# Juzhan/TAP-Net

Hardware: AMD Instinct MI355X
Metric: env-steps/s (batch placements) 2D n=10 LB_GREEDY; 1/2/4/8 GPU + CPU ref (higher is better)
Workload: dtype i32 height-maps / f64 candidate scores / f32 masks

## Files before the change

### tap-net_amd/csrc/tap_masks.h

```cpp
#pragma once

#include <hip/hip_runtime.h>

#include <cstdint>
#include <type_traits>
#include <cstdlib>

#include "tap_stream_variant.h"

constexpr size_t TAP_WT_MAX_BYTES = 64u << 20;

struct MaskArgs {
    int B, n, R, nR, rows, update_rows, static_rows;
    const float *dyn_in;
    float *dyn_out;
    const float *static_;
    const int64_t *ptr;
    const float *mask_in;
    const float *cs_in;
    float *cs_out;
    float *cur_out;
    float *mask_out;
    const unsigned long long *bits_in;
    unsigned long long *bits_out;
    int *nonbinary;
    int c4_magic, rp;
    int wt;
    int sb_mul, sb_add, nq, nq2;
    int inplace;
};

inline int tap_write_through(size_t bytes);

constexpr int TAP_HOT_MAGIC_MASK = 0xffffff, TAP_HOT_SB_MUL_SHIFT = 24, TAP_HOT_SB_ADD_SHIFT = 26, TAP_HOT_SB_MASK = 3;

inline MaskArgs mask_finish(MaskArgs a)
{
    const int c4 = a.nR >> 2;
    a.c4_magic = c4 > 0 ? 65536 / c4 + 1 : 0;
    static_assert(65536 + 1 <= TAP_HOT_MAGIC_MASK, "c4_magic shares its kernel argument with sb_mul / sb_add (TAP_MASK_HOT_ARGS)");
    a.rp = c4 > 0 ? 64 / c4 : 0;
    a.wt = tap_write_through((size_t)a.B * a.rows * a.nR * sizeof(float));
    const bool al = a.wt && c4 > 0 && ((a.rp * c4) & 3) == 0;
    a.sb_mul = al ? (a.rows * c4) & 3 : 0;
    a.sb_add = al ? (int)((reinterpret_cast<uintptr_t>(a.dyn_out) >> 4) & 3) : 0;
    a.nq = a.rp > 0 ? (a.rows + a.rp - 1) / a.rp : 0;
    a.nq2 = a.rp > 0 ? (2 * a.rows + a.rp - 1) / a.rp : 0;
    return a;
}

struct LaneRole {
    int rsub, c4;
    int r0;
    int nq;
    int sb;
};

__device__ __forceinline__ LaneRole stream_lane_role(int lane, int env, int C4, int RP, int c4_magic, int sb_mul, int sb_add, int nq)
{
    const int sb = __builtin_amdgcn_readfirstlane((env * sb_mul + sb_add) & 3);
    int role = lane - sb;
    const bool late = role < 0;
    role += late ? RP * C4 : 0;
    LaneRole o;
    o.rsub = (int)(((unsigned)role * (unsigned)c4_magic) >> 16);
    o.c4 = role - o.rsub * C4;
    o.r0 = o.rsub - (late ? RP : 0);
    o.nq = nq + (sb != 0);
    o.sb = sb;
    return o;
}

__host__ __device__ __forceinline__ bool mask_builds_bits(const MaskArgs &a) { return !a.bits_in && a.bits_out && a.dyn_in; }

#define TAP_MASK_HOT_PARAMS const int64_t *h_ptr, const float *h_static, const float *h_mask_in, const void *h_src, int h_B, \
                            int h_nR, int h_static_rows, int h_c4_magic
#define TAP_MASK_HOT_NAMES h_ptr, h_static, h_mask_in, h_src, h_B, h_nR, h_static_rows, h_c4_magic
#define TAP_MASK_HOT_ARGS(m) (m).ptr, (m).static_, (m).mask_in,                                                              \
        ((m).bits_in ? static_cast<const void *>((m).bits_in) : static_cast<const void *>((m).dyn_in)), (m).B, (m).nR,       \
        (m).static_rows, ((m).c4_magic | (((m).sb_mul & TAP_HOT_SB_MASK) << TAP_HOT_SB_MUL_SHIFT) |                           \
                          (((m).sb_add & TAP_HOT_SB_MASK) << TAP_HOT_SB_ADD_SHIFT))
__device__ __forceinline__ MaskArgs tap_mask_hot(const MaskArgs &k, bool src_is_bits, TAP_MASK_HOT_PARAMS)
{
    MaskArgs m = k;
    m.ptr = h_ptr; m.static_ = h_static; m.mask_in = h_mask_in;
    m.B = h_B; m.nR = h_nR; m.static_rows = h_static_rows; m.c4_magic = h_c4_magic & TAP_HOT_MAGIC_MASK;
    m.sb_mul = (h_c4_magic >> TAP_HOT_SB_MUL_SHIFT) & TAP_HOT_SB_MASK; m.sb_add = (h_c4_magic >> TAP_HOT_SB_ADD_SHIFT) & TAP_HOT_SB_MASK;
    if (src_is_bits) m.bits_in = static_cast<const unsigned long long *>(h_src);
    else m.dyn_in = static_cast<const float *>(h_src);
    return m;
}


#ifdef TAP_PROF
constexpr int TAP_PROF_WGS = 2048, TAP_PROF_WAVES = 16;
static __device__ unsigned long long tap_prof_tl[TAP_PROF_WGS * TAP_PROF_WAVES * 4];
#define TL_STAMP(i) do { if ((threadIdx.x & 63) == 0 && blockIdx.x < TAP_PROF_WGS) \
        tap_prof_tl[(blockIdx.x * TAP_PROF_WAVES + (threadIdx.x >> 6)) * 4 + (i)] = __builtin_amdgcn_s_memrealtime(); } while (0)
#define TL_WAIT_VM() __builtin_amdgcn_s_waitcnt(0)
#else
#define TL_STAMP(i) do { } while (0)
#define TL_WAIT_VM() do { } while (0)
#endif

__device__ __forceinline__ void tap_wave_lds_sync_m()
{
    __builtin_amdgcn_fence(__ATOMIC_RELEASE, "wavefront");
    __builtin_amdgcn_wave_barrier();
    __builtin_amdgcn_fence(__ATOMIC_ACQUIRE, "wavefront");
}

__device__ __forceinline__ void store_stream(float4 *dst, const float4 &v, int wt)
{
    typedef float v4f __attribute__((ext_vector_type(4)));
    const v4f nv = {v.x, v.y, v.z, v.w};
    if (wt) asm volatile("global_store_dwordx4 %0, %1, off sc0 sc1\n\ts_nop 1" : : "v"(dst), "v"(nv) : "memory");
    else __builtin_nontemporal_store(nv, reinterpret_cast<v4f *>(dst));
}

inline int tap_write_through(size_t bytes, size_t limit)
{
    static const int forced = [] { const char *e = getenv("TAP_WRITE_THROUGH"); return e ? (e[0] != '0') : -1; }();
    if (forced >= 0) return forced;
    return bytes <= limit;
}
inline int tap_write_through(size_t bytes) { return tap_write_through(bytes, TAP_WT_MAX_BYTES); }

__device__ __forceinline__ float bit_as_float(unsigned long long w, int r)
{
    const unsigned half = r < 32 ? (unsigned)w : (unsigned)(w >> 32);
    return (float)((half >> (r & 31)) & 1u);
}

__device__ __forceinline__ long tap_mod_col(long p, int n, int nR)
{
    if ((unsigned long)p >= (unsigned long)nR) p = 0;
    while (p >= n) p -= n;
    return p;
}

__device__ __forceinline__ void mask_column(const MaskArgs &a, int env, int j, long real_m,
                                            float move, float small, float large)
{
    float keep = a.mask_in ? a.mask_in[(size_t)env * a.nR + j] : 1.f;
    if (a.ptr)
        for (int r = 0; r < a.R; ++r)
            if (j == real_m + (long)a.n * r) keep = 0.f;
    if (a.mask_out) a.mask_out[(size_t)env * a.nR + j] = keep;
    const float dm = small * large + move;
    if (a.cur_out) a.cur_out[(size_t)env * a.nR + j] = dm != 0.f ? 0.f : keep;
}


struct ClearRanges {
    int lo[3], hi[3];
};

__device__ __forceinline__ ClearRanges clear_ranges(const MaskArgs &a, long real)
{
    ClearRanges c;
    for (int i = 0; i < 3; ++i) {
        const long r = real + (long)a.n * i;
        const bool on = i < a.update_rows && real >= 0 && r < a.rows;
        c.lo[i] = on ? (int)(r * a.nR) : -1;
        c.hi[i] = on ? (int)((r + 1) * a.nR) : -1;
    }
    return c;
}

__device__ __forceinline__ bool in_cleared(const ClearRanges &c, int f)
{
    return (f >= c.lo[0] && f < c.hi[0]) || (f >= c.lo[1] && f < c.hi[1]) || (f >= c.lo[2] && f < c.hi[2]);
}

__device__ __forceinline__ void mask_env(const MaskArgs &a, int env, int lane, long real, long p)
{
    const int nR = a.nR;
    const size_t slab = (size_t)a.rows * nR;
    const long real_m = (p >= 0 && p < nR) ? tap_mod_col(p, a.n, a.nR) : -1 - (long)a.n * a.R;
    for (int j = lane; j < nR; j += 64) {
        float sum[3], row[3];
#pragma unroll
        for (int s = 0; s < 3; ++s) {
            sum[s] = a.cs_in[((size_t)env * 3 + s) * nR + j];
            const long r = real + (long)a.n * s;
            row[s] = (a.dyn_out && s < a.update_rows && real >= 0 && r < a.rows)
                         ? a.dyn_in[(size_t)env * slab + (size_t)r * nR + j] : 0.f;
        }
#pragma unroll
        for (int s = 0; s < 3; ++s) {
            sum[s] -= row[s];
            if (a.cs_out) a.cs_out[((size_t)env * 3 + s) * nR + j] = sum[s];
        }
        mask_column(a, env, j, real_m, sum[0], sum[1], sum[2]);
    }
}

template <int NS, int U, int NC>
__device__ __forceinline__ void stream_wave_fast(const MaskArgs &a, int senv0, int lane,
                                                 const bool (&on)[NS], float *lds)
{
    const int nR = a.nR;
    const size_t slab = (size_t)a.rows * nR;
    const int nchunk = (int)(slab / 4);
    int total = 0;
#pragma unroll
    for (int k = 0; k < NS; ++k) if (on[k]) total = (k + 1) * nchunk;
    if (total == 0) return;
    long p[NS];
    float row0[NS][NC], cs[NS][NC][3], keep[NS][NC];
#pragma unroll
    for (int k = 0; k < NS; ++k) {
        const int env = senv0 + k;
        p[k] = on[k] ? (long)a.ptr[env] : 0;
#pragma unroll
        for (int c = 0; c < NC; ++c) {
            const int j = lane + 64 * c;
            const bool ok = on[k] && j < nR;
            row0[k][c] = ok ? a.static_[(size_t)env * a.static_rows * nR + j] : 0.f;
            keep[k][c] = ok ? (a.mask_in ? a.mask_in[(size_t)env * nR + j] : 1.f) : 0.f;
#pragma unroll
            for (int s = 0; s < 3; ++s) cs[k][c][s] = ok ? a.cs_in[((size_t)env * 3 + s) * nR + j] : 0.f;
        }
    }
    for (int i = lane; i < NS * 3 * nR; i += 64) lds[i] = 0.f;

    const float4 *s4 = reinterpret_cast<const float4 *>(a.dyn_in + (size_t)senv0 * slab);
    float4 *d4 = reinterpret_cast<float4 *>(a.dyn_out + (size_t)senv0 * slab);
    ClearRanges cr[NS];
    bool have_real = false;
    for (int base = 0; base < total; base += 64 * U) {
        float4 v[U];
#pragma unroll
        for (int u = 0; u < U; ++u) v[u] = s4[min(base + u * 64 + lane, total - 1)];
        if (!have_real) {
#pragma unroll
            for (int k = 0; k < NS; ++k) {
                float r0 = -1.f;
#pragma unroll
                for (int c = 0; c < NC; ++c) {
                    const float t = __shfl(row0[k][c], (int)(p[k] & 63));
                    if ((p[k] >> 6) == c && p[k] >= 0 && p[k] < nR) r0 = t;
                }
                cr[k] = clear_ranges(a, on[k] ? (long)r0 : -1);
            }
            have_real = true;
        }
#pragma unroll
        for (int u = 0; u < U; ++u) {
            const int q = base + u * 64 + lane;
            if (q < total) {
                const int k = (NS > 1 && q >= nchunk) ? 1 : 0;
                const int f = (q - k * nchunk) * 4;
#pragma unroll
                for (int s = 0; s < 3; ++s)
                    if (f >= cr[k].lo[s] && f < cr[k].hi[s]) {
                        *reinterpret_cast<float4 *>(lds + (k * 3 + s) * nR + (f - cr[k].lo[s])) = v[u];
                        v[u] = make_float4(0.f, 0.f, 0.f, 0.f);
                    }
                d4[q] = v[u];
            }
        }
    }
    __builtin_amdgcn_fence(__ATOMIC_RELEASE, "wavefront");
    __builtin_amdgcn_wave_barrier();
    __builtin_amdgcn_fence(__ATOMIC_ACQUIRE, "wavefront");
#pragma unroll
    for (int k = 0; k < NS; ++k) {
        if (!on[k]) continue;
        const int env = senv0 + k;
        const long real_m = (p[k] >= 0 && p[k] < nR) ? tap_mod_col(p[k], a.n, a.nR) : -1 - (long)a.n * a.R;
#pragma unroll
        for (int c = 0; c < NC; ++c) {
            const int j = lane + 64 * c;
            if (j >= nR) continue;
            float sum[3];
#pragma unroll
            for (int s = 0; s < 3; ++s) {
                sum[s] = cs[k][c][s] - lds[(k * 3 + s) * nR + j];
                if (a.cs_out) a.cs_out[((size_t)env * 3 + s) * nR + j] = sum[s];
            }
            float kp = keep[k][c];
            for (int r = 0; r < a.R; ++r)
                if (j == real_m + (long)a.n * r) kp = 0.f;
            if (a.mask_out) a.mask_out[(size_t)env * nR + j] = kp;
            const float dm = sum[1] * sum[2] + sum[0];
            if (a.cur_out) a.cur_out[(size_t)env * nR + j] = dm != 0.f ? 0.f : kp;
        }
    }
}

template <int NS>
__device__ __forceinline__ void stream_build_bits(const MaskArgs &a, int senv0, int lane, const bool (&on)[NS],
                                                  unsigned long long *tile )
{
    typedef unsigned long long u64;
    const int nR = a.nR, C4 = nR >> 2, rows = a.rows;
    const int rsub = (int)(((unsigned)lane * (unsigned)a.c4_magic) >> 16), c4 = lane - rsub * C4, RP = a.rp;
    for (int i = lane; i < NS * nR; i += 64) tile[i] = 0ull;
    tap_wave_lds_sync_m();
    int bad = 0;
    constexpr int U = 4;
    for (int r0 = rsub; r0 < rows; r0 += U * RP) {
        float4 v[NS][U];
#pragma unroll
        for (int k = 0; k < NS; ++k) {
            const float4 *src = reinterpret_cast<const float4 *>(a.dyn_in + (size_t)(senv0 + (on[k] ? k : 0)) * rows * nR) + c4;
#pragma unroll
            for (int u = 0; u < U; ++u) v[k][u] = src[(size_t)min(r0 + u * RP, rows - 1) * C4];
        }
#pragma unroll
        for (int k = 0; k < NS; ++k) {
            unsigned lo[4] = {0u, 0u, 0u, 0u}, hi[4] = {0u, 0u, 0u, 0u};
#pragma unroll
            for (int u = 0; u < U; ++u) {
                const int r = r0 + u * RP;
                if (r >= rows || rsub >= RP || !on[k]) continue;
                const float e[4] = {v[k][u].x, v[k][u].y, v[k][u].z, v[k][u].w};
#pragma unroll
                for (int q = 0; q < 4; ++q) {
                    const unsigned nz = e[q] != 0.f;
                    bad += (nz && e[q] != 1.f);
                    if (r < 32) lo[q] |= nz << r; else hi[q] |= nz << (r - 32);
                }
            }
            if (on[k] && rsub < RP) {
#pragma unroll
                for (int q = 0; q < 4; ++q) {
                    const u64 word = ((u64)hi[q] << 32) | lo[q];
                    if (word) atomicOr(&tile[k * nR + c4 * 4 + q], word);
                }
            }
        }
    }
    if (a.nonbinary) {
        const unsigned long long any = __ballot(bad != 0);
        if (any) {
#pragma unroll
            for (int o = 32; o > 0; o >>= 1) bad += __shfl_xor(bad, o);
            if (lane == 0) atomicAdd(a.nonbinary, bad);
        }
    }
    tap_wave_lds_sync_m();
}

__device__ __forceinline__ int tap_mod_small(int v, int n)
{
#pragma unroll
    for (int r = 0; r < 5; ++r) v = v >= n ? v - n : v;
    while (v >= n) v -= n;
    return v;
}

template <int NS, int NC, bool BUILD = false, bool MERGED = true, int C4S = 0, bool INPLACE = false, bool FULL = false>
__device__ __forceinline__ void stream_wave_bits_r4(const MaskArgs &a, int senv0, int lane, const bool (&on_)[NS],
                                                 float *lds = nullptr)
{
    static_assert(!(BUILD && INPLACE), "the first step on a fresh tensor writes all of it");
    bool on[NS];
#pragma unroll
    for (int k = 0; k < NS; ++k) on[k] = FULL ? true : on_[k];
#if defined(TAP_STREAM_LOAD_BJ)
    constexpr bool BJ_X = false;
#elif defined(TAP_STREAM_BJX_ALL)
    constexpr bool BJ_X = !BUILD && NC == 1 && (C4S == 5 || C4S == 15);
#else
    constexpr bool BJ_X = !BUILD && NC == 1 && NS == 1 && (C4S == 5 || C4S == 15);
#endif
    typedef unsigned long long u64;
    static_assert(NS <= 2, "a stream wave expands one or two slabs");
    if (!on[0]) return;
    const int nR = C4S ? 4 * C4S : a.nR, C4 = C4S ? C4S : nR >> 2, rows = C4S ? (C4S == 10 ? 60 : 30) : a.rows, n = C4S ? (C4S == 10 ? 20 : 10) : a.n;
    const int RP = C4S ? 64 / C4S : a.rp;
    const int c4_magic = C4S ? 65536 / C4S + 1 : a.c4_magic;
    const bool lane_on = lane < RP * C4;
#ifdef TAP_STREAM_UNALIGNED
    const LaneRole role = stream_lane_role(lane, 0, C4, RP, c4_magic, 0, 0, 0);
#else
    const LaneRole role = stream_lane_role(lane, senv0, C4, RP, c4_magic, a.sb_mul, a.sb_add, 0);
#endif
    const bool first_row = role.rsub == 0;
    u64 *tile = reinterpret_cast<u64 *>(lds);
    const void *any = BUILD ? static_cast<const void *>(a.dyn_in) : static_cast<const void *>(a.bits_in);
    const bool has_ptr = FULL || a.ptr != nullptr, has_static = FULL || a.static_ != nullptr, has_mask = FULL || a.mask_in != nullptr;
    const int64_t *ptrp = has_ptr ? a.ptr : static_cast<const int64_t *>(any);
    const float *stp = has_static ? a.static_ : static_cast<const float *>(any);
    const float *mip = has_mask ? a.mask_in : static_cast<const float *>(any);
    long praw[NS];
    float row0[NS][NC], keep[NS][NC];
    u64 bj[NS][NC];
    ulonglong2 w[NS][2];
#pragma unroll
    for (int k = 0; k < NS; ++k) {
        const int env = on[k] ? senv0 + k : senv0;
        praw[k] = ptrp[has_ptr ? env : 0];
        const float *strow = stp + (has_static ? (size_t)env * a.static_rows * nR : (size_t)0);
        const float *mirow = mip + (has_mask ? (size_t)env * nR : (size_t)0);
#pragma unroll
        for (int c = 0; c < NC; ++c) {
            const unsigned j = (unsigned)min(lane + 64 * c, nR - 1);
            row0[k][c] = strow[has_static ? j : 0u];
            keep[k][c] = mirow[has_mask ? j : 0u];
        }
    }
#ifdef TAP_STREAM_G2
    __builtin_amdgcn_s_waitcnt(0x0F70);
#endif
    if (!BUILD) {
#pragma unroll
        for (int k = 0; k < NS; ++k) {
            const int env = on[k] ? senv0 + k : senv0;
            const unsigned long long *brow = a.bits_in + (size_t)env * nR;
            if constexpr (!BJ_X) {
#pragma unroll
                for (int c = 0; c < NC; ++c) bj[k][c] = brow[(unsigned)min(lane + 64 * c, nR - 1)];
            }
            const ulonglong2 *src = reinterpret_cast<const ulonglong2 *>(brow) + (unsigned)(role.c4 * 2);
            w[k][0] = src[0];
            w[k][1] = src[1];
        }
    }
    if (BUILD) {
        stream_build_bits<NS>(a, senv0, lane, on, tile);
#pragma unroll
        for (int k = 0; k < NS; ++k) {
#pragma unroll
            for (int c = 0; c < NC; ++c) bj[k][c] = tile[(size_t)k * nR + min(lane + 64 * c, nR - 1)];
            const ulonglong2 *src = reinterpret_cast<const ulonglong2 *>(tile + (size_t)k * nR + role.c4 * 4);
            w[k][0] = src[0];
            w[k][1] = src[1];
        }
    }
    float *o_dyn = a.dyn_out, *o_cur = a.cur_out, *o_mask = a.mask_out;
    unsigned long long *o_bits = a.bits_out;
    int o_wt = a.wt;
#ifdef TAP_STREAM_EARLY_ARGS
    asm volatile("" : "+s"(o_dyn), "+s"(o_cur), "+s"(o_mask), "+s"(o_bits), "+s"(o_wt));
#endif
    __builtin_amdgcn_s_waitcnt(0x0F70);
#ifdef TAP_PROF
    TL_STAMP(1);
#endif
    const u64 nmask = (n >= 64) ? ~0ull : ((1ull << n) - 1ull);
    auto mod_n = [&](int v) -> int {
        if constexpr (C4S != 0) return (int)((unsigned)v % (unsigned)(C4S == 10 ? 20 : 10));
        else return tap_mod_small(v, n);
    };
    int jm[NC];
#pragma unroll
    for (int c = 0; c < NC; ++c) jm[c] = mod_n(min(lane + 64 * c, nR - 1));
    u64 clr[NS];
    int pm[NS], realk[NS];
    constexpr int UR_C = C4S != 0 ? 3 : 0;
    const int ur = UR_C ? UR_C : a.update_rows;
#pragma unroll
    for (int k = 0; k < NS; ++k) {
        const bool valid_v = on[k] && has_ptr && praw[k] >= 0 && praw[k] < nR;
#ifdef TAP_STREAM_VPICK
        constexpr bool SPICK = false;
#else
        constexpr bool SPICK = NS > 1;
#endif
        bool valid;
        int p, real;
        if constexpr (!SPICK) {
            valid = valid_v;
            p = valid ? (int)praw[k] : 0;
            float r0 = -1.f;
#pragma unroll
            for (int c = 0; c < NC; ++c) {
                const float t = __shfl(row0[k][c], p & 63);
                if (valid && has_static && (p >> 6) == c) r0 = t;
            }
            real = (r0 > -1.f && r0 < (float)rows) ? (int)r0 : -1;
        } else {
            const int ps = __builtin_amdgcn_readfirstlane(valid_v ? (int)praw[k] : -1);
            valid = ps >= 0;
            p = valid ? ps : 0;
            float r0 = -1.f;
#pragma unroll
            for (int c = 0; c < NC; ++c) {
                const float t = __int_as_float(__builtin_amdgcn_readlane(__float_as_int(row0[k][c]), p & 63));
                if (valid && has_static && (p >> 6) == c) r0 = t;
            }
            real = __builtin_amdgcn_readfirstlane((r0 > -1.f && r0 < (float)rows) ? (int)r0 : -1);
        }
        u64 m = 0;
#pragma unroll
        for (int i = 0; i < 3; ++i) {
            const int r = real + n * i;
            if (i < ur && real >= 0 && r < rows) m |= 1ull << r;
        }
        clr[k] = m;
        realk[k] = real;
        pm[k] = valid ? mod_n(p) : -1;
    }
    u64 nw[NS][4];
#pragma unroll
    for (int k = 0; k < NS; ++k) {
        nw[k][0] = w[k][0].x & ~clr[k]; nw[k][1] = w[k][0].y & ~clr[k];
        nw[k][2] = w[k][1].x & ~clr[k]; nw[k][3] = w[k][1].y & ~clr[k];
    }
    if constexpr (INPLACE) {
        if (o_dyn) {
            const float4 z = make_float4(0.f, 0.f, 0.f, 0.f);
            const int total = ur * C4;
            for (int idx = lane; idx < total; idx += 64) {
                const int i = (idx * c4_magic) >> 16, c = idx - i * C4;
#pragma unroll
                for (int k = 0; k < NS; ++k) {
                    const int r = realk[k] + n * i;
                    if (!on[k] || realk[k] < 0 || r >= rows) continue;
                    float4 *dst = reinterpret_cast<float4 *>(o_dyn) + ((size_t)(senv0 + k) * rows + r) * C4 + c;
#if defined(TAP_INPLACE_STORE) && TAP_INPLACE_STORE == 1
                    store_stream(dst, z, o_wt);
#elif defined(TAP_INPLACE_STORE) && TAP_INPLACE_STORE == 2
                    *dst = z;
#else
                    if (o_wt) store_stream(dst, z, 1); else *dst = z;
#endif
                }
            }
        }
    }
    if (lane_on) {
        if (!INPLACE && o_dyn) {
            const int non = (NS > 1 && on[NS - 1]) ? 2 : 1;
            const int total = non * rows;
            const int nq = (C4S ? (non * rows + RP - 1) / RP : (non > 1 ? a.nq2 : a.nq)) + role.nq;
            float4 *dst = reinterpret_cast<float4 *>(o_dyn + (size_t)senv0 * rows * nR) + role.c4;
            int rr = role.r0;
            bool done = false;
            if constexpr (NS > 1 && !MERGED) {
                if (rows <= 32) {
#pragma unroll
                    for (int k = 0; k < NS; ++k) {
                        if (!on[k]) continue;
                        float4 *dk = dst + (size_t)k * rows * C4;
                        const unsigned m0 = (unsigned)nw[k][0], m1 = (unsigned)nw[k][1], m2 = (unsigned)nw[k][2], m3 = (unsigned)nw[k][3];
                        for (int r = role.rsub; r < rows; r += RP) {
                            const float4 v = make_float4((float)((m0 >> r) & 1u), (float)((m1 >> r) & 1u),
                                                         (float)((m2 >> r) & 1u), (float)((m3 >> r) & 1u));
                            store_stream(&dk[(size_t)r * C4], v, o_wt);
                        }
                    }
                    done = true;
                }
            }
            if (done) {
            } else if (C4S != 0 && rows <= 32) {
                constexpr int ROWS_C = 30, RP_C = C4S ? 64 / C4S : 1, NQC = (NS * ROWS_C + RP_C - 1) / RP_C + 1;
                auto run = [&](auto wt_c) {
#pragma unroll
                    for (int i = 0; i < NQC; ++i) {
                        const int ri = rr + RP_C * i;
                        if ((unsigned)ri >= (unsigned)total) continue;
                        const bool up = NS > 1 && ri >= ROWS_C;
                        const int r = up ? ri - ROWS_C : ri;
                        const unsigned m0 = up ? (unsigned)nw[NS - 1][0] : (unsigned)nw[0][0], m1 = up ? (unsigned)nw[NS - 1][1] : (unsigned)nw[0][1],
                                       m2 = up ? (unsigned)nw[NS - 1][2] : (unsigned)nw[0][2], m3 = up ? (unsigned)nw[NS - 1][3] : (unsigned)nw[0][3];
                        const float4 v = make_float4((float)((m0 >> r) & 1u), (float)((m1 >> r) & 1u),
                                                     (float)((m2 >> r) & 1u), (float)((m3 >> r) & 1u));
                        store_stream(&dst[(size_t)ri * C4], v, decltype(wt_c)::value);
                    }
                };
#ifdef TAP_STREAM_ROLLED
                for (int i = 0; i < nq; ++i, rr += RP) {
                    if ((unsigned)rr >= (unsigned)total) continue;
                    const bool up = NS > 1 && rr >= rows;
                    const int r = up ? rr - rows : rr;
                    const unsigned m0 = up ? (unsigned)nw[NS - 1][0] : (unsigned)nw[0][0], m1 = up ? (unsigned)nw[NS - 1][1] : (unsigned)nw[0][1],
                                   m2 = up ? (unsigned)nw[NS - 1][2] : (unsigned)nw[0][2], m3 = up ? (unsigned)nw[NS - 1][3] : (unsigned)nw[0][3];
                    const float4 v = make_float4((float)((m0 >> r) & 1u), (float)((m1 >> r) & 1u),
                                                 (float)((m2 >> r) & 1u), (float)((m3 >> r) & 1u));
                    store_stream(&dst[(size_t)rr * C4], v, o_wt);
                }
#else
                if (o_wt) run(std::integral_constant<int, 1>{}); else run(std::integral_constant<int, 0>{});
#endif
            } else if (rows <= 32) {
                for (int i = 0; i < nq; ++i, rr += RP) {
                    if ((unsigned)rr >= (unsigned)total) continue;
                    const bool up = NS > 1 && rr >= rows;
                    const int r = up ? rr - rows : rr;
                    const unsigned m0 = up ? (unsigned)nw[NS - 1][0] : (unsigned)nw[0][0], m1 = up ? (unsigned)nw[NS - 1][1] : (unsigned)nw[0][1],
                                   m2 = up ? (unsigned)nw[NS - 1][2] : (unsigned)nw[0][2], m3 = up ? (unsigned)nw[NS - 1][3] : (unsigned)nw[0][3];
                    const float4 v = make_float4((float)((m0 >> r) & 1u), (float)((m1 >> r) & 1u),
                                                 (float)((m2 >> r) & 1u), (float)((m3 >> r) & 1u));
                    store_stream(&dst[(size_t)rr * C4], v, o_wt);
                }
            } else {
                for (int i = 0; i < nq; ++i, rr += RP) {
                    if ((unsigned)rr >= (unsigned)total) continue;
                    const bool up = NS > 1 && rr >= rows;
                    const int r = up ? rr - rows : rr;
                    const float4 v = make_float4(bit_as_float(up ? nw[NS - 1][0] : nw[0][0], r), bit_as_float(up ? nw[NS - 1][1] : nw[0][1], r),
                                                 bit_as_float(up ? nw[NS - 1][2] : nw[0][2], r), bit_as_float(up ? nw[NS - 1][3] : nw[0][3], r));
                    store_stream(&dst[(size_t)rr * C4], v, o_wt);
                }
            }
        }
        if (first_row && o_bits) {
#pragma unroll
            for (int k = 0; k < NS; ++k) {
                if (!on[k]) continue;
                ulonglong2 *dst = reinterpret_cast<ulonglong2 *>(o_bits + (size_t)(senv0 + k) * nR + role.c4 * 4);
                dst[0] = make_ulonglong2(nw[k][0], nw[k][1]);
                dst[1] = make_ulonglong2(nw[k][2], nw[k][3]);
            }
        }
    }
    unsigned nbx[NS];
    if constexpr (BJ_X) {
        const int jj = min(lane, nR - 1);
        const int src = ((jj >> 2) + role.sb) << 2;
        const int e = jj & 3;
#pragma unroll
        for (int k = 0; k < NS; ++k) {
            const int e0 = __builtin_amdgcn_ds_bpermute(src, (int)(unsigned)nw[k][0]), e1 = __builtin_amdgcn_ds_bpermute(src, (int)(unsigned)nw[k][1]);
            const int e2 = __builtin_amdgcn_ds_bpermute(src, (int)(unsigned)nw[k][2]), e3 = __builtin_amdgcn_ds_bpermute(src, (int)(unsigned)nw[k][3]);
            nbx[k] = (unsigned)(e == 0 ? e0 : e == 1 ? e1 : e == 2 ? e2 : e3);
        }
    }
#pragma unroll
    for (int k = 0; k < NS; ++k) {
        if (!on[k]) continue;
        const int env = senv0 + k;
#pragma unroll
        for (int c = 0; c < NC; ++c) {
            const int j = lane + 64 * c;
            if (j >= nR) continue;
            const u64 nb = BJ_X ? (u64)nbx[k] : (bj[k][c] & ~clr[k]);
            const int move = __popcll(nb & nmask), small = n >= 64 ? 0 : __popcll((nb >> n) & nmask);
            const int large = n >= 32 ? 0 : __popcll((nb >> (2 * n)) & nmask);
            const float kp = (jm[c] == pm[k]) ? 0.f : (has_mask ? keep[k][c] : 1.f);
            if (o_mask) o_mask[(size_t)env * nR + j] = kp;
            if (o_cur) o_cur[(size_t)env * nR + j] = (small * large + move) != 0 ? 0.f : kp;
        }
    }
}

#ifdef TAP_STREAM_R3
template <int NS, int NC, bool BUILD = false>
__device__ __forceinline__ void stream_wave_bits_r3(const MaskArgs &a, int senv0, int lane, const bool (&on)[NS],
                                                 float *lds = nullptr)
{
    typedef unsigned long long u64;
    const int nR = a.nR, C4 = nR >> 2, rows = a.rows;
    const int rsub = (int)(((unsigned)lane * (unsigned)a.c4_magic) >> 16), c4 = lane - rsub * C4, RP = a.rp;
    const bool lane_on = rsub < RP;
    constexpr bool build = BUILD;
    u64 *tile = reinterpret_cast<u64 *>(lds);
    long p[NS];
    float row0[NS][NC], keep[NS][NC];
    u64 bj[NS][NC];
    ulonglong2 w[NS][2];
#pragma unroll
    for (int k = 0; k < NS; ++k) {
        const int env = senv0 + k;
        p[k] = (on[k] && a.ptr) ? (long)a.ptr[env] : -1;
#pragma unroll
        for (int c = 0; c < NC; ++c) {
            const int j = lane + 64 * c;
            const bool ok = on[k] && j < nR;
            row0[k][c] = (ok && a.static_) ? a.static_[(size_t)env * a.static_rows * nR + j] : 0.f;
            keep[k][c] = ok ? (a.mask_in ? a.mask_in[(size_t)env * nR + j] : 1.f) : 0.f;
        }
    }
    if (BUILD) stream_build_bits<NS>(a, senv0, lane, on, tile);
#pragma unroll
    for (int k = 0; k < NS; ++k) {
        const int env = senv0 + k;
        const size_t wbase = build ? (size_t)k * nR : (size_t)env * nR;
#pragma unroll
        for (int c = 0; c < NC; ++c) {
            const int j = lane + 64 * c;
            const bool ok = on[k] && j < nR;
            if (BUILD) bj[k][c] = ok ? tile[wbase + j] : 0ull;
            else bj[k][c] = ok ? a.bits_in[wbase + j] : 0ull;
        }
        const bool ok = on[k] && lane_on;
        if (BUILD) {
            const ulonglong2 *src = reinterpret_cast<const ulonglong2 *>(tile + wbase + c4 * 4);
            w[k][0] = ok ? src[0] : make_ulonglong2(0, 0);
            w[k][1] = ok ? src[1] : make_ulonglong2(0, 0);
        } else {
            const ulonglong2 *src = reinterpret_cast<const ulonglong2 *>(a.bits_in + wbase + c4 * 4);
            w[k][0] = ok ? src[0] : make_ulonglong2(0, 0);
            w[k][1] = ok ? src[1] : make_ulonglong2(0, 0);
        }
    }
    const u64 nmask = (a.n >= 64) ? ~0ull : ((1ull << a.n) - 1ull);
#pragma unroll
    for (int k = 0; k < NS; ++k) {
        if (!on[k]) continue;
        const int env = senv0 + k;
        float r0 = -1.f;
#pragma unroll
        for (int c = 0; c < NC; ++c) {
            const float t = __shfl(row0[k][c], (int)(p[k] & 63));
            if ((p[k] >> 6) == c && p[k] >= 0 && p[k] < nR) r0 = t;
        }
        const long real = (long)r0;
        u64 clr = 0;
        for (int i = 0; i < a.update_rows; ++i) {
            const long r = real + (long)a.n * i;
            if (real >= 0 && r < rows) clr |= 1ull << r;
        }
        if (lane_on) {
            const u64 n0 = w[k][0].x & ~clr, n1 = w[k][0].y & ~clr, n2 = w[k][1].x & ~clr, n3 = w[k][1].y & ~clr;
#ifdef TAP_PROF
            if (k == 0) { TL_WAIT_VM(); TL_STAMP(1); }
#endif
            if (a.dyn_out) {
                float4 *dst = reinterpret_cast<float4 *>(a.dyn_out + (size_t)env * rows * nR) + c4;
                if (rows <= 32) {
                    const unsigned m0 = (unsigned)n0, m1 = (unsigned)n1, m2 = (unsigned)n2, m3 = (unsigned)n3;
                    for (int r = rsub; r < rows; r += RP) {
                        const float4 v = make_float4((float)((m0 >> r) & 1u), (float)((m1 >> r) & 1u),
                                                     (float)((m2 >> r) & 1u), (float)((m3 >> r) & 1u));
                        store_stream(&dst[(size_t)r * C4], v, a.wt);
                    }
                } else {
                    for (int r = rsub; r < rows; r += RP) {
                        const float4 v = make_float4(bit_as_float(n0, r), bit_as_float(n1, r), bit_as_float(n2, r),
                                                     bit_as_float(n3, r));
                        store_stream(&dst[(size_t)r * C4], v, a.wt);
                    }
                }
            }
            if (rsub == 0 && a.bits_out) {
                ulonglong2 *dst = reinterpret_cast<ulonglong2 *>(a.bits_out + (size_t)env * nR + c4 * 4);
                dst[0] = make_ulonglong2(n0, n1);
                dst[1] = make_ulonglong2(n2, n3);
            }
        }
        const long real_m = (p[k] >= 0 && p[k] < nR) ? tap_mod_col(p[k], a.n, a.nR) : -1 - (long)a.n * a.R;
#pragma unroll
        for (int c = 0; c < NC; ++c) {
            const int j = lane + 64 * c;
            if (j >= nR) continue;
            const u64 nb = bj[k][c] & ~clr;
            const int move = __popcll(nb & nmask), small = a.n >= 64 ? 0 : __popcll((nb >> a.n) & nmask);
            const int large = a.n >= 32 ? 0 : __popcll((nb >> (2 * a.n)) & nmask);
            float kp = keep[k][c];
            for (int r = 0; r < a.R; ++r)
                if (j == real_m + (long)a.n * r) kp = 0.f;
            if (a.mask_out) a.mask_out[(size_t)env * nR + j] = kp;
            if (a.cur_out) a.cur_out[(size_t)env * nR + j] = (small * large + move) != 0 ? 0.f : kp;
        }
    }
}

#endif
template <int NS, int NC, bool BUILD = false, bool MERGED = true, int C4S = 0, bool INPLACE = false, bool FULL = false>
__device__ __forceinline__ void stream_wave_bits(const MaskArgs &a, int senv0, int lane, const bool (&on)[NS], float *lds = nullptr)
{
#ifdef TAP_STREAM_R3
    stream_wave_bits_r3<NS, NC, BUILD>(a, senv0, lane, on, lds);
#else
    stream_wave_bits_r4<NS, NC, BUILD, MERGED, C4S, INPLACE, FULL>(a, senv0, lane, on, lds);
#endif
}

__host__ __device__ __forceinline__ int mask_bit_planes(int rows) { return rows > 64 ? 2 : 1; }

__device__ __forceinline__ unsigned long long bits_range64(int a, int b)
{
    a = a < 0 ? 0 : a;
    b = b > 64 ? 64 : b;
    if (a >= b) return 0ull;
    return ((b - a) >= 64 ? ~0ull : ((1ull << (b - a)) - 1ull)) << a;
}

template <int NC, bool BUILD>
__device__ __forceinline__ void stream_wave_bits2(const MaskArgs &a, int env, int lane, float *lds)
{
    typedef unsigned long long u64;
    const int nR = a.nR, C4 = nR >> 2, rows = a.rows;
    const int rsub = (int)(((unsigned)lane * (unsigned)a.c4_magic) >> 16), c4 = lane - rsub * C4, RP = a.rp;
    const bool lane_on = rsub < RP;
    u64 *tile = reinterpret_cast<u64 *>(lds);
    const long p = a.ptr ? (long)a.ptr[env] : -1;
    float row0[NC], keep[NC];
#pragma unroll
    for (int c = 0; c < NC; ++c) {
        const int j = lane + 64 * c;
        const bool ok = j < nR;
        row0[c] = (ok && a.static_) ? a.static_[(size_t)env * a.static_rows * nR + j] : 0.f;
        keep[c] = ok ? (a.mask_in ? a.mask_in[(size_t)env * nR + j] : 1.f) : 0.f;
    }
    if (BUILD) {
        for (int i = lane; i < 2 * nR; i += 64) tile[i] = 0ull;
        tap_wave_lds_sync_m();
        int bad = 0;
        constexpr int U = 4;
        const float4 *src = reinterpret_cast<const float4 *>(a.dyn_in + (size_t)env * rows * nR) + c4;
        u64 acc[2][4] = {{0ull, 0ull, 0ull, 0ull}, {0ull, 0ull, 0ull, 0ull}};
        for (int r0 = rsub; r0 < rows; r0 += U * RP) {
            float4 v[U];
#pragma unroll
            for (int u = 0; u < U; ++u) v[u] = src[(size_t)min(r0 + u * RP, rows - 1) * C4];
#pragma unroll
            for (int u = 0; u < U; ++u) {
                const int r = r0 + u * RP;
                if (r >= rows || !lane_on) continue;
                const float e[4] = {v[u].x, v[u].y, v[u].z, v[u].w};
#pragma unroll
                for (int q = 0; q < 4; ++q) {
                    const u64 nz = e[q] != 0.f;
                    bad += (nz && e[q] != 1.f);
                    if (r < 64) acc[0][q] |= nz << r; else acc[1][q] |= nz << (r - 64);
                }
            }
        }
        if (lane_on) {
#pragma unroll
            for (int w = 0; w < 2; ++w)
#pragma unroll
                for (int q = 0; q < 4; ++q)
                    if (acc[w][q]) atomicOr(&tile[w * nR + c4 * 4 + q], acc[w][q]);
        }
        if (a.nonbinary) {
            const unsigned long long any = __ballot(bad != 0);
            if (any) {
#pragma unroll
                for (int o = 32; o > 0; o >>= 1) bad += __shfl_xor(bad, o);
                if (lane == 0) atomicAdd(a.nonbinary, bad);
            }
        }
        tap_wave_lds_sync_m();
    }
    const u64 *win = BUILD ? tile : a.bits_in + (size_t)env * 2 * nR;
    const LaneRole role = stream_lane_role(lane, env, C4, RP, a.c4_magic, a.sb_mul, a.sb_add, a.nq);
    u64 bj[NC][2], w4[2][4];
#pragma unroll
    for (int c = 0; c < NC; ++c) {
        const int j = lane + 64 * c;
#pragma unroll
        for (int w = 0; w < 2; ++w) bj[c][w] = j < nR ? win[w * nR + j] : 0ull;
    }
#pragma unroll
    for (int w = 0; w < 2; ++w) {
        const ulonglong2 *src = reinterpret_cast<const ulonglong2 *>(win + w * nR + role.c4 * 4);
        const ulonglong2 s0 = lane_on ? src[0] : make_ulonglong2(0, 0), s1 = lane_on ? src[1] : make_ulonglong2(0, 0);
        w4[w][0] = s0.x; w4[w][1] = s0.y; w4[w][2] = s1.x; w4[w][3] = s1.y;
    }
    float r0 = -1.f;
#pragma unroll
    for (int c = 0; c < NC; ++c) {
        const float t = __shfl(row0[c], (int)(p & 63));
        if ((p >> 6) == c && p >= 0 && p < nR) r0 = t;
    }
    const long real = (long)r0;
    u64 clr[2] = {0ull, 0ull};
    for (int i = 0; i < a.update_rows; ++i) {
        const long r = real + (long)a.n * i;
        if (real >= 0 && r < rows) { if (r < 64) clr[0] |= 1ull << r; else clr[1] |= 1ull << (r - 64); }
    }
    if (lane_on) {
#pragma unroll
        for (int w = 0; w < 2; ++w)
#pragma unroll
            for (int q = 0; q < 4; ++q) w4[w][q] &= ~clr[w];
        if (a.dyn_out) {
            float4 *dst = reinterpret_cast<float4 *>(a.dyn_out + (size_t)env * rows * nR) + role.c4;
            int r = role.r0;
            for (int i = 0; i < role.nq; ++i, r += RP) {
                if ((unsigned)r >= (unsigned)rows) continue;
                const bool up = r >= 64;
                const int rb = r & 63;
                const float4 v = make_float4(bit_as_float(up ? w4[1][0] : w4[0][0], rb), bit_as_float(up ? w4[1][1] : w4[0][1], rb),
                                             bit_as_float(up ? w4[1][2] : w4[0][2], rb), bit_as_float(up ? w4[1][3] : w4[0][3], rb));
                store_stream(&dst[(size_t)r * C4], v, a.wt);
            }
        }
        if (role.rsub == 0 && a.bits_out) {
#pragma unroll
            for (int w = 0; w < 2; ++w) {
                ulonglong2 *dst = reinterpret_cast<ulonglong2 *>(a.bits_out + ((size_t)env * 2 + w) * nR + role.c4 * 4);
                dst[0] = make_ulonglong2(w4[w][0], w4[w][1]);
                dst[1] = make_ulonglong2(w4[w][2], w4[w][3]);
            }
        }
    }
    const long real_m = (p >= 0 && p < nR) ? tap_mod_col(p, a.n, a.nR) : -1 - (long)a.n * a.R;
    const int n = a.n;
#pragma unroll
    for (int c = 0; c < NC; ++c) {
        const int j = lane + 64 * c;
        if (j >= nR) continue;
        const u64 lo = bj[c][0] & ~clr[0], hi = bj[c][1] & ~clr[1];
        int sec[3];
#pragma unroll
        for (int s = 0; s < 3; ++s)
            sec[s] = __popcll(lo & bits_range64(s * n, (s + 1) * n)) + __popcll(hi & bits_range64(s * n - 64, (s + 1) * n - 64));
        float kp = keep[c];
        for (int r = 0; r < a.R; ++r)
            if (j == real_m + (long)n * r) kp = 0.f;
        if (a.mask_out) a.mask_out[(size_t)env * nR + j] = kp;
        if (a.cur_out) a.cur_out[(size_t)env * nR + j] = (sec[1] * sec[2] + sec[0]) != 0 ? 0.f : kp;
    }
}

inline bool mask_bits_ok(const MaskArgs &a)
{
    return (a.bits_in || mask_builds_bits(a)) && (a.ptr == nullptr || a.static_ != nullptr) && (a.nR % 4 == 0) &&
           a.nR <= 256 && a.rows >= 1 && a.rows <= 128 &&
           ((reinterpret_cast<uintptr_t>(a.dyn_out) | reinterpret_cast<uintptr_t>(a.dyn_in)) % 16 == 0) &&
           ((reinterpret_cast<uintptr_t>(a.bits_in) | reinterpret_cast<uintptr_t>(a.bits_out)) % 16 == 0);
}

inline int mask_fast_path_cols(const MaskArgs &a)
{
    if (a.bits_in || mask_builds_bits(a)) return a.nR <= 64 ? 1 : a.nR <= 128 ? 2 : 4;
    const bool ok = a.dyn_out && a.ptr && a.static_ && a.cs_in && (a.nR % 4 == 0) && a.nR <= 256 && a.rows >= 1 &&
                    ((reinterpret_cast<uintptr_t>(a.dyn_in) | reinterpret_cast<uintptr_t>(a.dyn_out)) % 16 == 0);
    return !ok ? 0 : a.nR <= 64 ? 1 : a.nR <= 128 ? 2 : 4;
}

inline TapMaskFacts tap_mask_facts(const MaskArgs &a)
{
    return TapMaskFacts{mask_fast_path_cols(a), a.bits_in ? 1 : mask_builds_bits(a) ? 2 : 0, a.inplace && a.dyn_out,
                        a.ptr && a.static_ && a.mask_in, a.wt != 0, a.n, a.rows, a.update_rows, a.nR};
}
```

Baseline: 1.484 billion.

## Stream dynamic tensor through registers on build step and vectorize mask/cur outputs

For the fixed-shape build path, the dense dynamic tensor is now loaded in chunks into registers, expanded and written out, and bit-packed in the same pass. This replaces the separate stream_build_bits tile construction; partial words are merged in LDS with atomicOr between wave syncs. The per-lane bj gathers and the bpermute path are removed. Mask and cur outputs are computed from the per-column-quad nw words and written as float4 stores by first-row lanes. This trades an extra LDS atomic merge and more register pressure for removing a second pass over the input.

```diff
diff --git a/tap-net_amd/csrc/tap_masks.h b/tap-net_amd/csrc/tap_masks.h
--- a/tap-net_amd/csrc/tap_masks.h
+++ b/tap-net_amd/csrc/tap_masks.h
@@ -360,12 +360,10 @@
     bool on[NS];
 #pragma unroll
     for (int k = 0; k < NS; ++k) on[k] = FULL ? true : on_[k];
-#if defined(TAP_STREAM_LOAD_BJ)
-    constexpr bool BJ_X = false;
-#elif defined(TAP_STREAM_BJX_ALL)
-    constexpr bool BJ_X = !BUILD && NC == 1 && (C4S == 5 || C4S == 15);
+#ifdef TAP_STREAM_BUILD_TILE
+    constexpr bool STREAM = false;
 #else
-    constexpr bool BJ_X = !BUILD && NC == 1 && NS == 1 && (C4S == 5 || C4S == 15);
+    constexpr bool STREAM = BUILD && C4S != 0;
 #endif
     typedef unsigned long long u64;
     static_assert(NS <= 2, "a stream wave expands one or two slabs");
@@ -386,9 +384,10 @@
     const int64_t *ptrp = has_ptr ? a.ptr : static_cast<const int64_t *>(any);
     const float *stp = has_static ? a.static_ : static_cast<const float *>(any);
     const float *mip = has_mask ? a.mask_in : static_cast<const float *>(any);
+    typedef float f4u __attribute__((ext_vector_type(4), aligned(4)));
     long praw[NS];
-    float row0[NS][NC], keep[NS][NC];
-    u64 bj[NS][NC];
+    float row0[NS][NC];
+    f4u keep[NS];
     ulonglong2 w[NS][2];
 #pragma unroll
     for (int k = 0; k < NS; ++k) {
@@ -400,8 +399,8 @@
         for (int c = 0; c < NC; ++c) {
             const unsigned j = (unsigned)min(lane + 64 * c, nR - 1);
             row0[k][c] = strow[has_static ? j : 0u];
-            keep[k][c] = mirow[has_mask ? j : 0u];
-        }
+        }
+        keep[k] = *reinterpret_cast<const f4u *>(mirow + (has_mask ? (unsigned)(role.c4 * 4) : 0u));
     }
 #ifdef TAP_STREAM_G2
     __builtin_amdgcn_s_waitcnt(0x0F70);
@@ -411,21 +410,15 @@
         for (int k = 0; k < NS; ++k) {
             const int env = on[k] ? senv0 + k : senv0;
             const unsigned long long *brow = a.bits_in + (size_t)env * nR;
-            if constexpr (!BJ_X) {
-#pragma unroll
-                for (int c = 0; c < NC; ++c) bj[k][c] = brow[(unsigned)min(lane + 64 * c, nR - 1)];
-            }
             const ulonglong2 *src = reinterpret_cast<const ulonglong2 *>(brow) + (unsigned)(role.c4 * 2);
             w[k][0] = src[0];
             w[k][1] = src[1];
         }
     }
-    if (BUILD) {
+    if constexpr (BUILD && !STREAM) {
         stream_build_bits<NS>(a, senv0, lane, on, tile);
 #pragma unroll
         for (int k = 0; k < NS; ++k) {
-#pragma unroll
-            for (int c = 0; c < NC; ++c) bj[k][c] = tile[(size_t)k * nR + min(lane + 64 * c, nR - 1)];
             const ulonglong2 *src = reinterpret_cast<const ulonglong2 *>(tile + (size_t)k * nR + role.c4 * 4);
             w[k][0] = src[0];
             w[k][1] = src[1];
@@ -437,7 +430,23 @@
 #ifdef TAP_STREAM_EARLY_ARGS
     asm volatile("" : "+s"(o_dyn), "+s"(o_cur), "+s"(o_mask), "+s"(o_bits), "+s"(o_wt));
 #endif
-    __builtin_amdgcn_s_waitcnt(0x0F70);
+    constexpr int ROWS_S = C4S == 10 ? 60 : 30, RP_S = C4S ? 64 / C4S : 1, C4_S = C4S ? C4S : 1, FL_S = C4S == 10 ? 4 : 9;
+    constexpr int NQ_S = (NS * ROWS_S + RP_S - 1) / RP_S + 1, NCH_S = (NQ_S + FL_S - 1) / FL_S, CH_S = (NQ_S + NCH_S - 1) / NCH_S;
+    const int s_total = ((NS > 1 && on[NS - 1]) ? 2 : 1) * ROWS_S;
+    float4 sv[CH_S];
+    auto s_row = [&](int i, int &ri) -> bool { ri = role.r0 + RP_S * i; return lane_on && (unsigned)ri < (unsigned)s_total; };
+    auto s_load = [&](int ch) {
+        const float4 *src = reinterpret_cast<const float4 *>(a.dyn_in + (size_t)senv0 * ROWS_S * nR) + role.c4;
+#pragma unroll
+        for (int u = 0; u < CH_S; ++u) {
+            int ri;
+            if (ch * CH_S + u >= NQ_S) continue;
+            const bool ok = s_row(ch * CH_S + u, ri);
+            sv[u] = src[ok ? (unsigned)(ri * C4_S) : 0u];
+        }
+    };
+    if constexpr (STREAM) s_load(0);
+    else __builtin_amdgcn_s_waitcnt(0x0F70);
 #ifdef TAP_PROF
     TL_STAMP(1);
 #endif
@@ -446,9 +455,9 @@
         if constexpr (C4S != 0) return (int)((unsigned)v % (unsigned)(C4S == 10 ? 20 : 10));
         else return tap_mod_small(v, n);
     };
-    int jm[NC];
-#pragma unroll
-    for (int c = 0; c < NC; ++c) jm[c] = mod_n(min(lane + 64 * c, nR - 1));
+    int jm[4];
+#pragma unroll
+    for (int q = 0; q < 4; ++q) jm[q] = mod_n(role.c4 * 4 + q);
     u64 clr[NS];
     int pm[NS], realk[NS];
     constexpr int UR_C = C4S != 0 ? 3 : 0;
@@ -496,10 +505,107 @@
         pm[k] = valid ? mod_n(p) : -1;
     }
     u64 nw[NS][4];
-#pragma unroll
-    for (int k = 0; k < NS; ++k) {
-        nw[k][0] = w[k][0].x & ~clr[k]; nw[k][1] = w[k][0].y & ~clr[k];
-        nw[k][2] = w[k][1].x & ~clr[k]; nw[k][3] = w[k][1].y & ~clr[k];
+    if constexpr (!STREAM) {
+#pragma unroll
+        for (int k = 0; k < NS; ++k) {
+            nw[k][0] = w[k][0].x & ~clr[k]; nw[k][1] = w[k][0].y & ~clr[k];
+            nw[k][2] = w[k][1].x & ~clr[k]; nw[k][3] = w[k][1].y & ~clr[k];
+        }
+    } else {
+        unsigned plo[NS][4], phi[NS][4];
+#pragma unroll
+        for (int k = 0; k < NS; ++k)
+#pragma unroll
+            for (int q = 0; q < 4; ++q) plo[k][q] = phi[k][q] = 0u;
+        int bad = 0;
+        float4 *dst = reinterpret_cast<float4 *>(o_dyn + (size_t)senv0 * ROWS_S * nR) + role.c4;
+        const bool expand = o_dyn != nullptr;
+        auto s_bits = [&](int ri, bool &up, unsigned &blo, unsigned &bhi) {
+            up = NS > 1 && ri >= ROWS_S;
+            const int r = up ? ri - ROWS_S : ri;
+            const u64 cw = up ? clr[NS - 1] : clr[0];
+            const bool high = ROWS_S > 32 && r >= 32;
+            const unsigned half = high ? (unsigned)(cw >> 32) : (unsigned)cw;
+            const unsigned bit = ((half >> (r & 31)) & 1u) ? 0u : 1u << (r & 31);
+            blo = high ? 0u : bit;
+            bhi = high ? bit : 0u;
+        };
+        auto s_chunk = [&](int ch, auto wt_c) {
+#pragma unroll
+            for (int u = 0; u < CH_S; ++u) {
+                int ri;
+                if (ch * CH_S + u >= NQ_S) continue;
+                if (!s_row(ch * CH_S + u, ri) || !expand) continue;
+                bool up;
+                unsigned blo, bhi;
+                s_bits(ri, up, blo, bhi);
+                const bool kept = (blo | bhi) != 0u;
+                const float4 o = make_float4((kept && sv[u].x != 0.f) ? 1.f : 0.f, (kept && sv[u].y != 0.f) ? 1.f : 0.f,
+                                             (kept && sv[u].z != 0.f) ? 1.f : 0.f, (kept && sv[u].w != 0.f) ? 1.f : 0.f);
+                store_stream(&dst[(size_t)ri * C4_S], o, decltype(wt_c)::value);
+            }
+#pragma unroll
+            for (int u = 0; u < CH_S; ++u) {
+                int ri;
+                if (ch * CH_S + u >= NQ_S) continue;
+                if (!s_row(ch * CH_S + u, ri)) continue;
+                bool up;
+                unsigned blo, bhi;
+                s_bits(ri, up, blo, bhi);
+                const float e[4] = {sv[u].x, sv[u].y, sv[u].z, sv[u].w};
+#pragma unroll
+                for (int q = 0; q < 4; ++q) {
+                    const bool nz = e[q] != 0.f;
+                    bad += (nz && e[q] != 1.f);
+#pragma unroll
+                    for (int k = 0; k < NS; ++k) {
+                        const bool mine = nz && (k == 0 ? !up : up);
+                        plo[k][q] |= mine ? blo : 0u;
+                        if (ROWS_S > 32) phi[k][q] |= mine ? bhi : 0u;
+                    }
+                }
+            }
+            if (ch + 1 < NCH_S) s_load(ch + 1);
+        };
+        auto s_run = [&](auto wt_c) {
+#pragma unroll
+            for (int ch = 0; ch < NCH_S; ++ch) s_chunk(ch, wt_c);
+        };
+        if (o_wt) s_run(std::integral_constant<int, 1>{}); else s_run(std::integral_constant<int, 0>{});
+        if (a.nonbinary) {
+            const unsigned long long any_bad = __ballot(bad != 0);
+            if (any_bad) {
+#pragma unroll
+                for (int o = 32; o > 0; o >>= 1) bad += __shfl_xor(bad, o);
+                if (lane == 0) atomicAdd(a.nonbinary, bad);
+            }
+        }
+        u64 *trow = tile + role.c4 * 4;
+        if (lane_on && first_row) {
+#pragma unroll
+            for (int k = 0; k < NS; ++k) {
+                ulonglong2 *t = reinterpret_cast<ulonglong2 *>(trow + (size_t)k * nR);
+                t[0] = make_ulonglong2(((u64)phi[k][0] << 32) | plo[k][0], ((u64)phi[k][1] << 32) | plo[k][1]);
+                t[1] = make_ulonglong2(((u64)phi[k][2] << 32) | plo[k][2], ((u64)phi[k][3] << 32) | plo[k][3]);
+            }
+        }
+        tap_wave_lds_sync_m();
+        if (lane_on && !first_row) {
+#pragma unroll
+            for (int k = 0; k < NS; ++k)
+#pragma unroll
+                for (int q = 0; q < 4; ++q) {
+                    const u64 word = ((u64)phi[k][q] << 32) | plo[k][q];
+                    if (word) atomicOr(&trow[(size_t)k * nR + q], word);
+                }
+        }
+        tap_wave_lds_sync_m();
+#pragma unroll
+        for (int k = 0; k < NS; ++k) {
+            const ulonglong2 *t = reinterpret_cast<const ulonglong2 *>(trow + (size_t)k * nR);
+            const ulonglong2 t0 = t[0], t1 = t[1];
+            nw[k][0] = t0.x; nw[k][1] = t0.y; nw[k][2] = t1.x; nw[k][3] = t1.y;
+        }
     }
     if constexpr (INPLACE) {
         if (o_dyn) {
@@ -524,7 +630,7 @@
         }
     }
     if (lane_on) {
-        if (!INPLACE && o_dyn) {
+        if (!STREAM && !INPLACE && o_dyn) {
             const int non = (NS > 1 && on[NS - 1]) ? 2 : 1;
             const int total = non * rows;
             const int nq = (C4S ? (non * rows + RP - 1) / RP : (non > 1 ? a.nq2 : a.nq)) + role.nq;
@@ -610,32 +716,22 @@
             }
         }
     }
-    unsigned nbx[NS];
-    if constexpr (BJ_X) {
-        const int jj = min(lane, nR - 1);
-        const int src = ((jj >> 2) + role.sb) << 2;
-        const int e = jj & 3;
+    if (lane_on && first_row) {
 #pragma unroll
         for (int k = 0; k < NS; ++k) {
-            const int e0 = __builtin_amdgcn_ds_bpermute(src, (int)(unsigned)nw[k][0]), e1 = __builtin_amdgcn_ds_bpermute(src, (int)(unsigned)nw[k][1]);
-            const int e2 = __builtin_amdgcn_ds_bpermute(src, (int)(unsigned)nw[k][2]), e3 = __builtin_amdgcn_ds_bpermute(src, (int)(unsigned)nw[k][3]);
-            nbx[k] = (unsigned)(e == 0 ? e0 : e == 1 ? e1 : e == 2 ? e2 : e3);
-        }
-    }
-#pragma unroll
-    for (int k = 0; k < NS; ++k) {
-        if (!on[k]) continue;
-        const int env = senv0 + k;
-#pragma unroll
-        for (int c = 0; c < NC; ++c) {
-            const int j = lane + 64 * c;
-            if (j >= nR) continue;
-            const u64 nb = BJ_X ? (u64)nbx[k] : (bj[k][c] & ~clr[k]);
-            const int move = __popcll(nb & nmask), small = n >= 64 ? 0 : __popcll((nb >> n) & nmask);
-            const int large = n >= 32 ? 0 : __popcll((nb >> (2 * n)) & nmask);
-            const float kp = (jm[c] == pm[k]) ? 0.f : (has_mask ? keep[k][c] : 1.f);
-            if (o_mask) o_mask[(size_t)env * nR + j] = kp;
-            if (o_cur) o_cur[(size_t)env * nR + j] = (small * large + move) != 0 ? 0.f : kp;
+            if (!on[k]) continue;
+            f4u kp, cu;
+#pragma unroll
+            for (int q = 0; q < 4; ++q) {
+                const u64 nb = nw[k][q];
+                const int move = __popcll(nb & nmask), small = n >= 64 ? 0 : __popcll((nb >> n) & nmask);
+                const int large = n >= 32 ? 0 : __popcll((nb >> (2 * n)) & nmask);
+                kp[q] = (jm[q] == pm[k]) ? 0.f : (has_mask ? keep[k][q] : 1.f);
+                cu[q] = (small * large + move) != 0 ? 0.f : kp[q];
+            }
+            const size_t at = (size_t)(senv0 + k) * nR + role.c4 * 4;
+            if (o_mask) *reinterpret_cast<f4u *>(o_mask + at) = kp;
+            if (o_cur) *reinterpret_cast<f4u *>(o_cur + at) = cu;
         }
     }
 }
```

New measurement: 1.357 billion. -8.6%, worse.
